# Schaudge/cellranger

Measured on AMD Instinct MI355X. Metric: M reads/sec barcode-correct+UMI-count, higher is better.
Workload: dtype u32/u64 integer keys; f64 posterior

## Files before the change

cellranger_amd/csrc/dedup.hip:

```cpp
#include "block_utils.h"
#include "common.h"

int cr_scan_small(crgpu_ctx *ctx, uint32_t *d_data, uint64_t n, uint32_t *d_total_out);
int cr_partition_by_owner(crgpu_ctx *ctx, const uint64_t *d_in, uint64_t *d_out, uint64_t n, uint32_t sh_bc,
                          uint32_t n_ranks, const uint32_t *bounds, uint64_t *counts_out);

#define NONE32 0xFFFFFFFFu

struct crgpu_counts {
    uint64_t n_triplets = 0, n_molecules = 0;
    uint32_t *d_bc = nullptr, *d_feature = nullptr, *d_count = nullptr;
    uint64_t *d_mkeys = nullptr;
    uint32_t *d_mreads = nullptr;
    uint32_t *d_corr_reads = nullptr;
    uint32_t *d_filt_reads = nullptr;
    int32_t *d_mprobe = nullptr;
    uint32_t *d_back = nullptr;
    uint32_t n_back = 0;
    uint32_t n_canon = 0;
    KeyLayout layout;
    bool pt_valid = false;
    uint32_t pt_n_probes = 0;
    uint64_t n_pt = 0;
    uint32_t *d_pt_bc = nullptr, *d_pt_probe = nullptr, *d_pt_count = nullptr;
// ... 709 lines not shown
}
__device__ __forceinline__ uint32_t rep_source(uint32_t min_raw, uint32_t K, uint32_t sK) {
    return (min_raw != 0xFFFFFFFFu && (min_raw < K || (sK & ST_CORRECTED))) ? min_raw : 0xFFFFFFFFu;
}

struct TargetFilter {
    const uint8_t *on_target;
    uint32_t n_features, sh_feat, bits_feat;
    uint64_t min_reads;
    __device__ __forceinline__ bool filtered(uint64_t key, uint32_t read_count, bool low) const {
        if (!min_reads) return false;
        const uint32_t f = (uint32_t)((key >> sh_feat) & lowmask(bits_feat));
        return f < n_features && on_target[f] != 0 && (uint64_t)read_count < min_reads && !low;
    }
};
struct MolFlag {
    const uint16_t *st;
    __device__ __forceinline__ bool operator()(uint64_t k) const {
        const uint32_t s = st[k];
        const bool landed = !(s & ST_CORRECTED) | (st_inc1(s) > 0u);
        return landed & !(s & ST_LOW);
    }
};
struct MolFlagTargeted {
    const uint16_t *st;
    const uint64_t *ukey;
    const uint32_t *upos, *inc_all;
    uint64_t n_keys, n_dist;
    TargetFilter tf;
    __device__ __forceinline__ bool operator()(uint64_t k) const {
        const uint32_t s = st[k];
        const bool landed = !(s & ST_CORRECTED) | (st_inc1(s) > 0u);
        if (!landed || (s & ST_LOW)) return false;
        const uint32_t end = k + 1 < n_dist ? upos[k + 1] : (uint32_t)n_keys;
        const uint32_t rc = ((s & ST_CORRECTED) ? 0u : end - upos[k]) + (st_inc1(s) ? inc_all[k] : 0u);
        return !tf.filtered(ukey[k], rc, false);
    }
};
struct EmitMol {
    const uint64_t *ukey;
    const uint32_t *upos, *inc_all, *minidx;
    const uint16_t *st;
    uint64_t n_keys, n_dist;
    uint64_t *mkeys;
    uint32_t *mreads;
    const uint32_t *rep_read = nullptr;
    const int32_t *probe = nullptr;
    int32_t *mprobe = nullptr;
    struct Pre {
        uint64_t key;
        uint32_t p0, p1, s;
    };
    __device__ __forceinline__ Pre pre(uint64_t k) const {
        Pre p;
        p.key = ukey[k];
        p.p0 = upos[k];
        p.p1 = upos[k + 1 < n_dist ? k + 1 : k];
        p.s = st[k];
        return p;
    }
    __device__ __forceinline__ Pre pre_own(uint64_t k) const {
        Pre p;
        p.key = ukey[k];
        p.p0 = upos[k];
        p.p1 = 0u;
        p.s = st[k];
        return p;
    }
    __device__ __forceinline__ void operator()(uint64_t k, uint32_t o, const Pre &p) const {
        uint32_t inc = 0u, mi = NONE32;
        if (st_inc1(p.s)) {
            inc = inc_all[k];
            mi = rep_source(minidx[k], (uint32_t)k, p.s);
        }
        const uint64_t bit = (mi != NONE32 ? ukey[mi] : p.key) & 1ull;
        mkeys[o] = (p.key & ~1ull) | bit;
        const uint32_t end = k + 1 < n_dist ? p.p1 : (uint32_t)n_keys;
        const uint32_t cnt = end - p.p0;
        mreads[o] = ((p.s & ST_CORRECTED) ? 0u : cnt) + inc;
        if (mprobe) mprobe[o] = probe[rep_read[mi != NONE32 ? mi : (uint32_t)k]];
    }
};

__device__ __forceinline__ bool rl_is_head(uint64_t key, uint64_t &carry_key, bool &carry_valid, uint32_t shift, uint32_t lane) {
    uint64_t left = __shfl_up(key, 1);
    if (lane == 0) left = carry_key;
    const bool head = (lane == 0 && !carry_valid) || (key >> shift) != (left >> shift);
    carry_key = __shfl(key, 63);
    carry_valid = true;
    return head;
}

__global__ __launch_bounds__(CP_BLOCK) void k_rl_count(const uint64_t *__restrict__ keys, const uint32_t shift, const uint64_t n,
                                                       const uint64_t tile, uint32_t *__restrict__ block_counts) {
    __shared__ uint32_t ws[CP_WAVES];
    const uint32_t lane = threadIdx.x & 63u, wave = threadIdx.x >> 6;
    const uint64_t lo = (uint64_t)blockIdx.x * tile;
    const uint64_t hi = lo + tile < n ? lo + tile : n;
    uint32_t c = 0;
    for (uint64_t base = lo; base < hi; base += CP_ROUND) {
        uint64_t key[CP_ITEMS];
        const uint64_t w0 = base + (uint64_t)wave * (64u * CP_ITEMS);
        const uint64_t wb = w0 > 0 ? (w0 - 1 < n ? w0 - 1 : n - 1) : 0;
        uint64_t carry_key = keys[wb];
        bool carry_valid = w0 > 0;
#pragma unroll
        for (int j = 0; j < CP_ITEMS; j++) {
            const uint64_t i = w0 + (uint64_t)j * 64 + lane;
            key[j] = keys[i < hi ? i : hi - 1];
        }
#pragma unroll
        for (int j = 0; j < CP_ITEMS; j++) {
            const uint64_t i = w0 + (uint64_t)j * 64 + lane;
            const bool head = rl_is_head(key[j], carry_key, carry_valid, shift, lane);
            c += (head && i < hi) ? 1u : 0u;
        }
    }
#pragma unroll
    for (int d = 32; d >= 1; d >>= 1) c += __shfl_xor(c, d);
    if (lane == 0) ws[wave] = c;
    __syncthreads();
    if (threadIdx.x == 0) {
        uint32_t t = 0;
        for (int w = 0; w < CP_WAVES; w++) t += ws[w];
        block_counts[blockIdx.x] = t;
    }
}

__global__ __launch_bounds__(CP_BLOCK) void k_rl_write(const uint64_t *__restrict__ keys, const uint32_t shift, const uint64_t n,
                                                       const uint64_t tile, const uint32_t *__restrict__ block_offs,
                                                       uint64_t *__restrict__ ukey, uint32_t *__restrict__ upos) {
    __shared__ uint32_t ws[CP_ITEMS * CP_WAVES];
    __shared__ uint32_t round_total;
    const uint32_t lane = threadIdx.x & 63u, wave = threadIdx.x >> 6;
    const uint64_t lo = (uint64_t)blockIdx.x * tile;
    const uint64_t hi = lo + tile < n ? lo + tile : n;
    uint32_t run = block_offs[blockIdx.x];
    for (uint64_t base = lo; base < hi; base += CP_ROUND) {
        uint64_t key[CP_ITEMS];
        bool f[CP_ITEMS];
        uint32_t below[CP_ITEMS];
        const uint64_t w0 = base + (uint64_t)wave * (64u * CP_ITEMS);
        const uint64_t wb = w0 > 0 ? (w0 - 1 < n ? w0 - 1 : n - 1) : 0;
        uint64_t carry_key = keys[wb];
        bool carry_valid = w0 > 0;
#pragma unroll
        for (int j = 0; j < CP_ITEMS; j++) {
            const uint64_t i = w0 + (uint64_t)j * 64 + lane;
            key[j] = keys[i < hi ? i : hi - 1];
        }
#pragma unroll
        for (int j = 0; j < CP_ITEMS; j++) {
            const uint64_t i = w0 + (uint64_t)j * 64 + lane;
            f[j] = rl_is_head(key[j], carry_key, carry_valid, shift, lane) && i < hi;
            const unsigned long long m = __ballot(f[j]);
            below[j] = (uint32_t)__popcll(m & ((1ull << lane) - 1ull));
            if (lane == 0) ws[wave * CP_ITEMS + j] = (uint32_t)__popcll(m);
        }
        __syncthreads();
        if (threadIdx.x < CP_ITEMS * CP_WAVES) {
            const uint32_t v = ws[threadIdx.x];
            uint32_t x = v;
#pragma unroll
            for (int d = 1; d < CP_ITEMS * CP_WAVES; d <<= 1) {
                const uint32_t y = __shfl_up(x, d);
                if (threadIdx.x >= (uint32_t)d) x += y;
            }
            ws[threadIdx.x] = x - v;
            if (threadIdx.x == CP_ITEMS * CP_WAVES - 1) round_total = x;
        }
        __syncthreads();
#pragma unroll
        for (int j = 0; j < CP_ITEMS; j++)
            if (f[j]) {
                const uint32_t o = run + ws[wave * CP_ITEMS + j] + below[j];
                ukey[o] = key[j];
                upos[o] = (uint32_t)(w0 + (uint64_t)j * 64 + lane);
            }
        run += round_total;
        __syncthreads();
    }
}

static int run_lengths(crgpu_ctx *ctx, const uint64_t *keys, uint32_t shift, uint64_t n, uint64_t *ukey, uint32_t *upos,
                       uint32_t *d_block, uint32_t *d_total_out, bool counts_ready = false) {
    uint64_t tile;
    const uint32_t nb = cp_blocks(n, &tile);
    if (!counts_ready)
        hipLaunchKernelGGL(k_rl_count, dim3(nb), dim3(CP_BLOCK), 0, ctx->stream, keys, shift, n, tile, d_block);
    else
        ctx->rl_counts_from_finish++;
    CR_TRY(cr_scan_small(ctx, d_block, nb, d_total_out));
    hipLaunchKernelGGL(k_rl_write, dim3(nb), dim3(CP_BLOCK), 0, ctx->stream, keys, shift, n, tile, d_block, ukey, upos);
    CR_HIP(ctx, hipGetLastError());
    return CRGPU_OK;
}

struct MtCarry {
    uint64_t prefix;
    bool has_mol;
    bool valid;
};

template <typename Flag>
__device__ __forceinline__ MtCarry mt_carry_from_memory(const Flag &flag, const uint64_t *__restrict__ ukey, uint32_t sh_feat,
                                                        uint64_t nd, uint64_t i0) {
    MtCarry c{0ull, false, false};
    if (i0 == 0 || i0 >= nd) return c;
    c.valid = true;
    uint64_t p = i0 - 1;
    c.prefix = ukey[p] >> sh_feat;
    c.has_mol = flag(p);
    while (!c.has_mol && p > 0) {
        p--;
        if ((ukey[p] >> sh_feat) != c.prefix) break;
        c.has_mol = flag(p);
    }
    return c;
}

__device__ __forceinline__ bool mt_opens_triplet(bool is_mol, uint64_t key, uint32_t sh_feat, uint32_t lane, MtCarry &carry) {
    const uint64_t prefix = key >> sh_feat;
    const uint64_t left = __shfl_up(prefix, 1);
    const unsigned long long starts = __ballot(lane == 0 || prefix != left), mols = __ballot(is_mol);
    const unsigned long long upto = ~0ull >> (63u - lane);
    const uint32_t rs = 63u - (uint32_t)__clzll((long long)(starts & upto));
    const unsigned long long between = (upto >> 1) & ~((1ull << rs) - 1ull);
    const uint64_t prefix0 = __shfl(prefix, 0);
    const bool carried = carry.valid && carry.prefix == prefix0 && carry.has_mol;
    const bool open = (mols & between) == 0ull && !(rs == 0u && carried);
    const uint32_t rs_last = 63u - (uint32_t)__clzll((long long)starts);
    const bool last_has = (mols >> rs_last) != 0ull || (rs_last == 0u && carried);
    carry.prefix = __shfl(prefix, 63);
    carry.has_mol = last_has;
    carry.valid = true;
    return is_mol && open;
}

#define MT_WAVE_SPAN (64u * CP_ITEMS)
template <typename Flag>
__global__ __launch_bounds__(CP_BLOCK) void k_mt_count(const Flag flag, const uint64_t *__restrict__ ukey, const uint32_t sh_feat,
                                                       const uint64_t nd, const uint64_t tile, uint32_t *__restrict__ mol_counts,
                                                       uint32_t *__restrict__ head_counts) {
    __shared__ uint32_t ws[2 * CP_WAVES];
    const uint32_t lane = threadIdx.x & 63u, wave = threadIdx.x >> 6;
    const uint64_t lo = (uint64_t)blockIdx.x * tile;
    const uint64_t hi = lo + tile < nd ? lo + tile : nd;
    uint32_t cm = 0, ch = 0;
    for (uint64_t base = lo; base < hi; base += CP_ROUND) {
        bool f[CP_ITEMS];
        uint64_t key[CP_ITEMS];
        const uint64_t w0 = base + (uint64_t)wave * MT_WAVE_SPAN;
#pragma unroll
        for (int j = 0; j < CP_ITEMS; j++) {
            const uint64_t i = w0 + (uint64_t)j * 64 + lane;
            const uint64_t ic = i < hi ? i : hi - 1;
            f[j] = flag(ic);
            key[j] = ukey[ic];
        }
        MtCarry carry = mt_carry_from_memory(flag, ukey, sh_feat, nd, w0);
#pragma unroll
        for (int j = 0; j < CP_ITEMS; j++) {
            const uint64_t i = w0 + (uint64_t)j * 64 + lane;
            const bool m = f[j] && i < hi;
            const bool h = mt_opens_triplet(m, key[j], sh_feat, lane, carry);
            cm += m ? 1u : 0u;
            ch += h ? 1u : 0u;
        }
    }
#pragma unroll
    for (int d = 32; d >= 1; d >>= 1) {
        cm += __shfl_xor(cm, d);
        ch += __shfl_xor(ch, d);
    }
    if (lane == 0) {
        ws[wave] = cm;
// ... 70 lines not shown
            ws[threadIdx.x] = x - v;
            if (threadIdx.x == CP_ITEMS * CP_WAVES - 1) round_total = x;
        }
        __syncthreads();
#pragma unroll
        for (int j = 0; j < CP_ITEMS; j++)
            if (f[j]) {
                const uint64_t i = w0 + (uint64_t)j * 64 + lane;
                const uint32_t w = ws[wave * CP_ITEMS + j];
                const uint32_t o = run_m + (w & 0xFFFFu) + below_m[j];
                emit(i, o, pre[j]);
                if (h[j]) {
                    const uint32_t t = run_h + (w >> 16) + below_h[j];
                    const uint32_t bcf = (uint32_t)(pre[j].key >> sh_bc);
                    tbc[t] = back ? back[bcf] : bcf;
                    tfeat[t] = (uint32_t)((pre[j].key >> sh_feat) & lowmask(bits_feat));
                    tpos[t] = o;
                }
            }
        run_m += round_total & 0xFFFFu;
        run_h += round_total >> 16;
        __syncthreads();
    }
}

__global__ __launch_bounds__(256) void k_trip_counts(const uint32_t *__restrict__ tpos, uint64_t nt, uint64_t nm,
                                                     uint32_t *__restrict__ cnt) {
    const uint64_t stride = (uint64_t)gridDim.x * blockDim.x;
    for (uint64_t t = (uint64_t)blockIdx.x * blockDim.x + threadIdx.x; t < nt; t += stride)
        cnt[t] = (t + 1 < nt ? tpos[t + 1] : (uint32_t)nm) - tpos[t];
}

__device__ __forceinline__ void segment_bounds(const uint64_t *__restrict__ ukey, uint64_t nd, uint64_t k, uint32_t shift,
                                               uint64_t &s, uint64_t &e) {
    const uint64_t pre = ukey[k] >> shift;
    uint64_t lo = k, step = 1;
    while (lo >= step && (ukey[lo - step] >> shift) == pre) {
        lo -= step;
        step <<= 1;
    }
    uint64_t a = lo >= step ? lo - step + 1 : 0, b = lo;
    while (a < b) {
        const uint64_t mid = (a + b) >> 1;
        if ((ukey[mid] >> shift) == pre) b = mid; else a = mid + 1;
    }
    s = a;
    uint64_t hi = k;
    step = 1;
    while (hi + step < nd && (ukey[hi + step] >> shift) == pre) {
        hi += step;
        step <<= 1;
    }
    a = hi;
    b = hi + step < nd ? hi + step - 1 : nd - 1;
    while (a < b) {
        const uint64_t mid = (a + b + 1) >> 1;
        if ((ukey[mid] >> shift) == pre) a = mid; else b = mid - 1;
    }
    e = a + 1;
}

__device__ __forceinline__ uint32_t run_count(const uint32_t *__restrict__ upos, uint64_t nd, uint64_t n_keys, uint64_t k) {
    const uint32_t end = k + 1 < nd ? upos[k + 1] : (uint32_t)n_keys;
    return end - upos[k];
}

#include "umi_correct.h"

__device__ __forceinline__ uint64_t group_id(const KL &kl, uint64_t key) {
    const uint64_t umi = (key >> kl.sh_umi) & lowmask(kl.bits_umi);
    const uint64_t lib = (key >> kl.sh_lib) & lowmask(kl.bits_lib + kl.bits_ulen);
    const uint64_t bc = key >> kl.sh_bc;
    return ((bc << (kl.bits_lib + kl.bits_ulen)) | lib) << kl.bits_umi | umi;
}
__device__ __forceinline__ uint32_t group_hash(uint64_t g) {
    g ^= g >> 33;
    g *= 0xff51afd7ed558ccdull;
    g ^= g >> 33;
    g *= 0xc4ceb9fe1a85ec53ull;
    g ^= g >> 33;
    return (uint32_t)g;
}

#define LF_TILE 8192u
#define LF_ENTRY_BITS 18u
#define LF_WORDS (1u << (LF_ENTRY_BITS - 4u))
__device__ __forceinline__ uint64_t mix64(uint64_t g) {
    g ^= g >> 33;
    g *= 0xff51afd7ed558ccdull;
    g ^= g >> 33;
    g *= 0xc4ceb9fe1a85ec53ull;
    g ^= g >> 33;
    return g;
}
#define LF_THREADS 1024u
#define LF_BATCH 4
#define LS_HASH_BITS 32u
__device__ __forceinline__ void lf_note(uint32_t *bm, uint32_t e) {
    const uint32_t sh = (e & 15u) * 2u;
    const uint32_t old = atomicOr(&bm[e >> 4], 1u << sh);
    if ((old >> sh) & 1u) atomicOr(&bm[e >> 4], 2u << sh);
}
__device__ __forceinline__ bool lf_again(const uint32_t *bm, uint32_t e) { return (bm[e >> 4] >> ((e & 15u) * 2u + 1u)) & 1u; }
__global__ __launch_bounds__(LF_THREADS) void k_group_candidates(const KL kl, const uint64_t *__restrict__ ukey, uint64_t nd,
                                                                 uint8_t *__restrict__ cand) {
    __shared__ uint32_t bm[LF_WORDS];
    __shared__ uint32_t s_first;
    __shared__ unsigned long long s_end;
    const uint32_t tid = threadIdx.x;
    const uint64_t n_tiles = (nd + LF_TILE - 1) / LF_TILE;
    const uint32_t emask = (1u << LF_ENTRY_BITS) - 1u;
    for (uint64_t tile = blockIdx.x; tile < n_tiles; tile += gridDim.x) {
        const uint64_t t0 = tile * LF_TILE;
        const uint64_t t1 = t0 + LF_TILE < nd ? t0 + LF_TILE : nd;
        if (tid == 0) s_first = 0xFFFFFFFFu;
        for (uint32_t w = tid; w < LF_WORDS; w += LF_THREADS) bm[w] = 0u;
        __syncthreads();
        {
            uint32_t mine = 0xFFFFFFFFu;
#pragma unroll
            for (uint32_t j = 0; j < LF_TILE / LF_THREADS; j++) {
                const uint64_t p = t0 + j * LF_THREADS + tid;
                if (p < t1 && mine == 0xFFFFFFFFu && (p == 0 || (ukey[p] >> kl.sh_bc) != (ukey[p - 1] >> kl.sh_bc)))
                    mine = (uint32_t)(p - t0);
            }
            if (mine != 0xFFFFFFFFu) atomicMin(&s_first, mine);
        }
        __syncthreads();
        const uint32_t first = s_first;
        if (tid == 0) {
            uint64_t b = nd;
            if (first != 0xFFFFFFFFu && t1 < nd) {
                const uint64_t bcv = ukey[t1 - 1] >> kl.sh_bc;
                uint64_t lo = t1 - 1, step = 1;
                while (lo + step < nd && (ukey[lo + step] >> kl.sh_bc) == bcv) {
                    lo += step;
                    step <<= 1;
                }
                uint64_t hi = lo + step < nd ? lo + step : nd;
                while (lo + 1 < hi) {
                    const uint64_t mid = (lo + hi) >> 1;
                    if ((ukey[mid] >> kl.sh_bc) == bcv) lo = mid; else hi = mid;
                }
                b = hi;
            }
            s_end = b;
        }
        __syncthreads();
        if (first == 0xFFFFFFFFu) continue;
        const uint64_t a = t0 + first, b = s_end;
        for (uint64_t k0 = a + tid; k0 < b; k0 += (uint64_t)LF_THREADS * LF_BATCH) {
            uint64_t key[LF_BATCH];
#pragma unroll
            for (int j = 0; j < LF_BATCH; j++) {
                const uint64_t k = k0 + (uint64_t)j * LF_THREADS;
                key[j] = k < b ? ukey[k] : 0ull;
            }
#pragma unroll
            for (int j = 0; j < LF_BATCH; j++) {
                if (k0 + (uint64_t)j * LF_THREADS >= b) break;
                lf_note(bm, (uint32_t)mix64(group_id(kl, key[j])) & emask);
            }
        }
        __syncthreads();
        for (uint64_t k0 = a + tid; k0 < b; k0 += (uint64_t)LF_THREADS * LF_BATCH) {
            uint64_t key[LF_BATCH];
#pragma unroll
            for (int j = 0; j < LF_BATCH; j++) {
                const uint64_t k = k0 + (uint64_t)j * LF_THREADS;
                key[j] = k < b ? ukey[k] : 0ull;
            }
#pragma unroll
            for (int j = 0; j < LF_BATCH; j++) {
                const uint64_t k = k0 + (uint64_t)j * LF_THREADS;
                if (k >= b) break;
                cand[k] = (uint8_t)lf_again(bm, (uint32_t)mix64(group_id(kl, key[j])) & emask);
            }
        }
        __syncthreads();
    }
}
struct CandFlag {
    const uint8_t *cand;
    __device__ __forceinline__ bool operator()(uint64_t k) const { return cand[k] != 0; }
};
struct EmitHash {
    KL kl;
    const uint64_t *ukey;
    uint32_t vbits;
    uint32_t *hash, *val;
    typedef uint64_t Pre;
    __device__ __forceinline__ Pre pre(uint64_t k) const { return ukey[k]; }
    __device__ __forceinline__ void operator()(uint64_t k, uint32_t o, Pre key) const {
        const uint64_t g = mix64(group_id(kl, key) ^ 0x9E3779B97F4A7C15ull);
        hash[o] = LS_HASH_BITS >= 32u ? (uint32_t)g : ((uint32_t)g & ((1u << (LS_HASH_BITS & 31u)) - 1u));
        const uint32_t extra = vbits >= 32u ? 0u : ((uint32_t)(g >> 32) << vbits);
        val[o] = extra | (uint32_t)k;
    }
};

__global__ __launch_bounds__(256) void k_low_support(const KL kl, const uint32_t *__restrict__ hash,
                                                     const uint32_t *__restrict__ val, uint64_t n_cand, uint64_t nd,
                                                     uint32_t vbits,
                                                     const uint64_t *__restrict__ ukey,
                                                     const uint32_t *__restrict__ upos, uint64_t n_keys,
                                                     uint16_t *__restrict__ st) {
    const uint64_t stride = (uint64_t)gridDim.x * blockDim.x;
    for (uint64_t j = (uint64_t)blockIdx.x * blockDim.x + threadIdx.x; j < n_cand; j += stride) {
        const uint32_t h = hash[j];
        const bool same_prev = j > 0 && hash[j - 1] == h;
        const bool same_next = j + 1 < n_cand && hash[j + 1] == h;
        if (!same_prev && !same_next) continue;
        uint64_t s = j, e = j + 1;
        while (s > 0 && hash[s - 1] == h) s--;
        while (e < n_cand && hash[e] == h) e++;
        const uint32_t vmask = vbits >= 32u ? 0xFFFFFFFFu : ((1u << vbits) - 1u);
        const uint32_t my_val = val[j];
        bool any = false;
        for (uint64_t t = s; t < e; t++) any |= t != j && ((val[t] ^ my_val) & ~vmask) == 0u;
        if (!any) continue;
        const uint32_t me = my_val & vmask;
        const uint64_t g = group_id(kl, ukey[me]);
        const uint32_t my_s = st[me];
        const uint32_t my_c1 = run_count(upos, nd, n_keys, me) - ((my_s & ST_CORRECTED) ? 1u : 0u) + st_inc1(my_s);
        uint32_t mx = my_c1, n_members = 0, n_max = 0;
        for (uint64_t t = s; t < e; t++) {
            if (((val[t] ^ my_val) & ~vmask) != 0u) continue;
            const uint32_t k = val[t] & vmask;
            if (group_id(kl, ukey[k]) != g) continue;
            const uint32_t ks = st[k];
            const uint32_t c1 = run_count(upos, nd, n_keys, k) - ((ks & ST_CORRECTED) ? 1u : 0u) + st_inc1(ks);
            n_members++;
            if (c1 > mx) {
                mx = c1;
                n_max = 1;
            } else if (c1 == mx) {
                n_max++;
            }
        }
        if (n_members < 2) continue;
        if (my_c1 < mx || n_max >= 2) st_or(st, me, ST_LOW);
    }
}

__global__ __launch_bounds__(256) void k_rep_read(const uint64_t *__restrict__ keys, const uint32_t *__restrict__ vals,
                                                  const uint32_t *__restrict__ upos, uint64_t nd, uint64_t n_keys,
                                                  uint32_t *__restrict__ rep_read) {
    const uint64_t stride = (uint64_t)gridDim.x * blockDim.x;
    for (uint64_t k = (uint64_t)blockIdx.x * blockDim.x + threadIdx.x; k < nd; k += stride) {
        const uint32_t b = upos[k], e = k + 1 < nd ? upos[k + 1] : (uint32_t)n_keys;
        const uint64_t bit = keys[b] & 1ull;
        uint32_t best = vals[b];
        for (uint32_t i = b + 1; i < e && (keys[i] & 1ull) == bit; i++) best = vals[i] < best ? vals[i] : best;
        rep_read[k] = best;
    }
}

struct __attribute__((aligned(4))) DupRec {
    uint32_t umi, read_count, flags;
};

struct __attribute__((aligned(8))) DupRec8 {
    uint32_t umi_flags, read_count;
};
template <bool PACK8>
__global__ __launch_bounds__(256) void k_per_read(const KL kl, const uint64_t *__restrict__ ukey, const uint32_t *__restrict__ vals,
                                                  const uint32_t *__restrict__ upos, uint64_t nd, uint64_t n_keys,
                                                  const uint32_t *__restrict__ corr, const uint32_t *__restrict__ inc_all,
                                                  const uint16_t *__restrict__ st, const uint32_t *__restrict__ minidx,
                                                  const uint32_t *__restrict__ rep_read, void *__restrict__ packed_v,
                                                  const TargetFilter tf) {
    DupRec *__restrict__ packed = reinterpret_cast<DupRec *>(packed_v);
    DupRec8 *__restrict__ packed8 = reinterpret_cast<DupRec8 *>(packed_v);
    const uint64_t stride = (uint64_t)gridDim.x * blockDim.x;
    for (uint64_t k = (uint64_t)blockIdx.x * blockDim.x + threadIdx.x; k < nd; k += stride) {
        const uint32_t b = upos[k], e = k + 1 < nd ? upos[k + 1] : (uint32_t)n_keys;
        const bool corrected = (st[k] & ST_CORRECTED) != 0u;
        const uint32_t K = corrected ? corr[k] : (uint32_t)k;
        const uint32_t sK = st[K];
        const uint32_t endK = (uint64_t)K + 1 < nd ? upos[K + 1] : (uint32_t)n_keys;
        const uint32_t cntK = endK - upos[K];
        const bool is_target = st_inc1(sK) != 0u;
// ... 205 lines not shown
            ctx->timing = was_timing;
        }
        if (t0) {
            ctx->event_pool.push_back(t0);
            ctx->event_pool.push_back(t1);
        }
    }
};

static int count_keys_impl(crgpu_ctx *ctx, uint64_t *d_keys_inout, uint64_t n_keys, crgpu_counts **out, PerRead pr) {
    if (!ctx || !out) return CRGPU_EINVAL;
    *out = nullptr;
    CR_REQUIRE(ctx, ctx->layout.set, CRGPU_ESTATE, "crgpu_count_keys: call crgpu_set_key_layout first");
    CR_REQUIRE(ctx, n_keys <= 0x7FFFFFFFull, CRGPU_ERANGE, "crgpu_count_keys: at most 2^31-1 keys per call");
    CR_TRY(cr_dense_ensure(ctx));
    const KeyLayout &L = ctx->layout;
    const KL kl = make_kl(L);
    crgpu_counts *res = new (std::nothrow) crgpu_counts();
    if (!res) return cr_fail(ctx, CRGPU_ENOMEM, "out of host memory");
    res->layout = L;
    res->n_canon = ctx->n_canon;
    if (n_keys == 0) {
        *out = res;
        return CRGPU_OK;
    }
    CR_REQUIRE(ctx, L.total_bits() <= 64, CRGPU_ESTATE,
               "crgpu_count_keys: the key layout needs the dense barcode index (CRGPU_OPT_DENSE_BARCODE_KEYS) and none is valid -- "
               "were the keys built before the last change of a histogram table?");
    CR_REQUIRE(ctx, d_keys_inout, CRGPU_EINVAL, "crgpu_count_keys: NULL keys");
    struct Guard {
        crgpu_ctx *c;
        crgpu_counts *r;
        bool armed = true;
        ~Guard() {
            if (armed) crgpu_counts_free(c, r);
        }
    } guard{ctx, res};

    uint32_t *d_block = ctx->d_sort_hist;
    uint32_t *d_total = ctx->d_scalars + 16;
    if (ctx->dense.valid) {
        res->n_back = ctx->dense.V;
        CR_TRY(cr_pool_alloc(ctx, (void **)&res->d_back, (size_t)ctx->dense.V * sizeof(uint32_t)));
        CR_HIP(ctx, hipMemcpyAsync(res->d_back, ctx->dense.d_back, (size_t)ctx->dense.V * sizeof(uint32_t), hipMemcpyDeviceToDevice,
                                   ctx->stream));
    }

    DevBuf tmp, vtmp;
    CR_TRY(dmalloc(ctx, tmp, n_keys * sizeof(uint64_t)));
    if (pr.d_vals) CR_TRY(dmalloc(ctx, vtmp, n_keys * sizeof(uint32_t)));
    bool in_tmp = false;
    uint32_t low_left = 0;
    CR_TRY(cr_radix_sort_u64_top(ctx, d_keys_inout, tmp.as<uint64_t>(), pr.d_vals, pr.d_vals ? vtmp.as<uint32_t>() : nullptr, n_keys,
                                 L.total_bits(), &in_tmp, &low_left));
    uint64_t *keys_rw = in_tmp ? tmp.as<uint64_t>() : d_keys_inout;
    uint32_t *vals_rw = pr.d_vals ? (in_tmp ? vtmp.as<uint32_t>() : pr.d_vals) : nullptr;

    DevBuf ukey_b, upos_b;
    CR_TRY(dmalloc(ctx, ukey_b, n_keys * sizeof(uint64_t)));
    CR_TRY(dmalloc(ctx, upos_b, (n_keys + 1) * sizeof(uint32_t)));
    uint64_t *ukey = ukey_b.as<uint64_t>();
    uint32_t *upos = upos_b.as<uint32_t>();
    CrRunHeads rl_heads{1u, 0, d_block, false};
    if (low_left) {
        bool fell_back = false;
        (void)cp_blocks(n_keys, &rl_heads.tile);
        CR_TRY(cr_order_runs(ctx, keys_rw, vals_rw, n_keys, low_left, &fell_back, &rl_heads));
        if (fell_back) {
            ctx->sort_refinished++;
            uint64_t *other = in_tmp ? d_keys_inout : tmp.as<uint64_t>();
            uint32_t *vother = pr.d_vals ? (in_tmp ? pr.d_vals : vtmp.as<uint32_t>()) : nullptr;
            bool flip = false;
            CR_TRY(cr_radix_sort_u64_full(ctx, keys_rw, other, vals_rw, vother, n_keys, L.total_bits(), &flip));
            if (flip) {
                keys_rw = other;
                vals_rw = vother;
            }
            rl_heads.valid = false;
        }
    }
    const uint64_t *keys = keys_rw;
    const uint32_t *vals = vals_rw;
    uint32_t nd32 = 0;
    {
        CrTimer t(ctx, CRGPU_T_DEDUP, n_keys);
        CR_TRY(run_lengths(ctx, keys, 1u, n_keys, ukey, upos, d_block, d_total, rl_heads.valid));
    }
    CR_TRY(read_u32(ctx, d_total, &nd32));
    const uint64_t nd = nd32;

    const uint64_t st_bytes = ((nd + 1) & ~1ull) * sizeof(uint16_t) + 4;
    DevBuf corr_b, incall_b, st_b, minidx_b;
    CR_TRY(dmalloc(ctx, minidx_b, nd * sizeof(uint32_t)));
    CR_TRY(dmalloc(ctx, corr_b, nd * sizeof(uint32_t)));
    CR_TRY(dmalloc(ctx, incall_b, nd * sizeof(uint32_t)));
    CR_TRY(dmalloc(ctx, st_b, st_bytes));
    uint32_t *corr = corr_b.as<uint32_t>(), *inc_all = incall_b.as<uint32_t>(), *minidx = minidx_b.as<uint32_t>();
    uint16_t *st = st_b.as<uint16_t>();
    const bool overlap = CrFork::enabled(ctx, nd);
    CrFork fork(ctx);
    DevBuf heads_b, giant_b, best_b;
    if (overlap) CR_TRY(fork.mark());
    {
        const bool timing_was = ctx->timing;
        if (overlap) ctx->timing = false;
        struct TimingBack {
            crgpu_ctx *c;
            bool v;
            ~TimingBack() { c->timing = v; }
        } timing_back{ctx, timing_was};
        CrTimer t(ctx, CRGPU_T_DEDUP);
        CR_HIP(ctx, hipMemsetAsync(inc_all, 0, nd * sizeof(uint32_t), ctx->stream));
        CR_HIP(ctx, hipMemsetAsync(st, 0, st_bytes, ctx->stream));
        CR_HIP(ctx, hipMemsetAsync(minidx, 0xFF, nd * sizeof(uint32_t), ctx->stream));
        const uint64_t n_tiles = (nd + UC_TILE - 1) / UC_TILE;
        CR_TRY(dmalloc(ctx, heads_b, 2 * n_tiles * sizeof(uint32_t)));
        uint32_t *tile_first = heads_b.as<uint32_t>(), *tile_last = tile_first + n_tiles;
#ifndef UC_GRID_WG
#define UC_GRID_WG 5u
#endif
        hipLaunchKernelGGL(k_correct_umis_tiled, dim3(cr_grid(n_tiles, 1, 256u * UC_GRID_WG)), dim3(256), 0, ctx->stream, kl, ukey,
                           upos, nd, n_keys, tile_first, tile_last, corr, st, inc_all, minidx);
        if (n_tiles > 1) {
            const size_t lds_small = (2 * UES_CAP + UES_BUCKETS * 8) * sizeof(uint32_t);
            const size_t lds_large = (2 * UE_CAP + UE_BUCKETS * 8) * sizeof(uint32_t);
            cr_allow_lds(ctx, (const void *)k_correct_umis_edges<false>, lds_large);
            cr_allow_lds(ctx, (const void *)k_giant_probe, lds_large);
            const uint64_t max_items = nd / (UE_CAP / 2) + 16;
            CR_TRY(dmalloc(ctx, giant_b, max_items * sizeof(GiantItem) + 16));
            CR_TRY(dmalloc(ctx, best_b, nd * sizeof(unsigned long long)));
            uint32_t *n_giant = reinterpret_cast<uint32_t *>(giant_b.as<unsigned char>());
            GiantItem *items = reinterpret_cast<GiantItem *>(giant_b.as<unsigned char>() + 16);
            unsigned long long *best = best_b.as<unsigned long long>();
            CR_HIP(ctx, hipMemsetAsync(n_giant, 0, sizeof(uint32_t), ctx->stream));
            hipLaunchKernelGGL(k_correct_umis_edges<true>, dim3(cr_grid(n_tiles - 1, 1, 256u * 6u)), dim3(UES_THREADS), lds_small,
                               ctx->stream, kl, ukey, upos, nd, n_keys, tile_first, tile_last, corr, st, inc_all, minidx, items, n_giant);
            hipLaunchKernelGGL(k_correct_umis_edges<false>, dim3(cr_grid(n_tiles - 1, 1, 256u * 2u)), dim3(UE_THREADS),
                               lds_large, ctx->stream, kl, ukey, upos, nd, n_keys, tile_first, tile_last, corr, st, inc_all,
                               minidx, items, n_giant);
            hipLaunchKernelGGL(k_giant_init, dim3(512), dim3(UE_THREADS), 0, ctx->stream, kl, ukey, upos, nd, n_keys, items,
                               n_giant, best);
            hipLaunchKernelGGL(k_giant_probe, dim3(512), dim3(UE_THREADS), lds_large, ctx->stream, kl, ukey, upos, nd, n_keys,
                               items, n_giant, best);
            hipLaunchKernelGGL(k_giant_final, dim3(512), dim3(UE_THREADS), 0, ctx->stream, upos, nd, n_keys, items, n_giant, best,
                               corr, st, inc_all, minidx);
        }
        CR_HIP(ctx, hipGetLastError());
    }

    {
        DevBuf cand_b, h_b, v_b;
        CR_TRY(dmalloc(ctx, cand_b, nd));
        CR_TRY(dmalloc(ctx, h_b, nd * sizeof(uint32_t)));
        CR_TRY(dmalloc(ctx, v_b, nd * sizeof(uint32_t)));
        const uint32_t vbits = cr_ceil_log2(nd ? nd : 1);
        uint32_t n_cand32 = 0;
        if (overlap) CR_TRY(fork.side(fork.t0));
        {
            CrTimer t(ctx, CRGPU_T_DEDUP);
            const uint64_t n_ftiles = (nd + LF_TILE - 1) / LF_TILE;
            hipLaunchKernelGGL(k_group_candidates, dim3(cr_grid(n_ftiles, 1, 256u * 2u)), dim3(LF_THREADS), 0, ctx->stream, kl, ukey, nd,
                               cand_b.as<uint8_t>());
            CR_HIP(ctx, hipGetLastError());
            CR_TRY(compact(ctx, CandFlag{cand_b.as<uint8_t>()}, EmitHash{kl, ukey, vbits, h_b.as<uint32_t>(), v_b.as<uint32_t>()}, nd, d_block,
                           d_total));
        }
        CR_TRY(read_u32(ctx, d_total, &n_cand32));
        const uint64_t n_cand = n_cand32;
        ctx->last_distinct_keys = nd;
        ctx->last_low_support_candidates = n_cand;
        if (n_cand >= 2) {
            DevBuf ht_b, vt_b;
            CR_TRY(dmalloc(ctx, ht_b, n_cand * sizeof(uint32_t)));
            CR_TRY(dmalloc(ctx, vt_b, n_cand * sizeof(uint32_t)));
            bool s_in_tmp = false;
            CR_TRY(cr_radix_sort_u32(ctx, h_b.as<uint32_t>(), ht_b.as<uint32_t>(), v_b.as<uint32_t>(), vt_b.as<uint32_t>(), n_cand,
                                     0, LS_HASH_BITS, &s_in_tmp));
            CR_TRY(fork.join());
            {
                CrTimer t(ctx, CRGPU_T_DEDUP);
                hipLaunchKernelGGL(k_low_support, dim3(cr_grid(n_cand, 256)), dim3(256), 0, ctx->stream, kl,
                                   s_in_tmp ? ht_b.as<uint32_t>() : h_b.as<uint32_t>(),
                                   s_in_tmp ? vt_b.as<uint32_t>() : v_b.as<uint32_t>(), n_cand, nd, vbits, ukey, upos, n_keys, st);
                CR_HIP(ctx, hipGetLastError());
            }
        }
        CR_TRY(fork.join());
    }

    const TargetFilter tf{ctx->d_on_target, ctx->n_target_features, L.sh_feat(), L.bits_feat, ctx->d_on_target ? ctx->target_min_reads : 0};
    CrFork fork2(ctx);
    DevBuf rep_b, packed_b;
    const bool want_probe = vals && pr.d_probe;
    if (vals) CR_TRY(dmalloc(ctx, rep_b, nd * sizeof(uint32_t)));
    if (want_probe) {
        CrTimer t(ctx, CRGPU_T_DEDUP);
        hipLaunchKernelGGL(k_rep_read, dim3(cr_grid(nd, 256)), dim3(256), 0, ctx->stream, keys, vals, upos, nd, n_keys,
                           rep_b.as<uint32_t>());
        CR_HIP(ctx, hipGetLastError());
    }
    if (vals && CrFork::enabled(ctx, nd)) {
        CR_TRY(fork2.mark());
        CR_TRY(fork2.side(fork2.t0));
    }
    const uint32_t side_wgs = fork2.on_side ? 256u * 6u : 256u * 8u;
    if (vals) {
        CrTimer t(ctx, CRGPU_T_DEDUP);
        if (!want_probe)
            hipLaunchKernelGGL(k_rep_read, dim3(cr_grid(nd, 256, side_wgs)), dim3(256), 0, ctx->stream, keys, vals, upos, nd, n_keys,
                               rep_b.as<uint32_t>());
        if (pr.packed_out) CR_HIP(ctx, hipMemsetAsync(pr.packed_out, 0, pr.n_reads * sizeof(DupRec), ctx->stream));
        const bool pack8 = !pr.packed_out && kl.bits_umi <= 24u;
        if (!pr.packed_out) {
            const uint64_t bytes = pr.n_reads * (pack8 ? sizeof(DupRec8) : sizeof(DupRec));
            CR_TRY(dmalloc(ctx, packed_b, bytes));
            CR_HIP(ctx, hipMemsetAsync(packed_b.p, 0, bytes, ctx->stream));
        }
        DupRec *packed = pr.packed_out ? pr.packed_out : packed_b.as<DupRec>();
        if (pack8)
            hipLaunchKernelGGL(k_per_read<true>, dim3(cr_grid(nd, 256, side_wgs)), dim3(256), 0, ctx->stream, kl, ukey, vals, upos, nd, n_keys,
                               corr, inc_all, st, minidx, rep_b.as<uint32_t>(), (void *)packed, tf);
        else
            hipLaunchKernelGGL(k_per_read<false>, dim3(cr_grid(nd, 256, side_wgs)), dim3(256), 0, ctx->stream, kl, ukey, vals, upos, nd, n_keys,
                               corr, inc_all, st, minidx, rep_b.as<uint32_t>(), (void *)packed, tf);
        if (!pr.packed_out) {
            if (pack8)
                hipLaunchKernelGGL(k_unpack_dupinfo<true>, dim3(cr_grid(pr.n_reads, 256, side_wgs)), dim3(256), 0, ctx->stream,
                                   (const void *)packed, pr.n_reads, pr.out_umi, pr.out_cnt, pr.out_flags);
            else
                hipLaunchKernelGGL(k_unpack_dupinfo<false>, dim3(cr_grid(pr.n_reads, 256, side_wgs)), dim3(256), 0, ctx->stream,
                                   (const void *)packed, pr.n_reads, pr.out_umi, pr.out_cnt, pr.out_flags);
        }
        CR_HIP(ctx, hipGetLastError());
    }
    fork2.pause();

    DevBuf mkeys_b, mreads_b, tpos_b;
    CR_TRY(dmalloc(ctx, mkeys_b, nd * sizeof(uint64_t)));
    CR_TRY(dmalloc(ctx, mreads_b, nd * sizeof(uint32_t)));
    uint32_t nm32 = 0, nt32 = 0;
    if (want_probe) CR_TRY(cr_pool_alloc(ctx, (void **)&res->d_mprobe, nd * sizeof(int32_t)));
    CR_TRY(dmalloc(ctx, tpos_b, (nd + 1) * sizeof(uint32_t)));
    CR_TRY(cr_pool_alloc(ctx, (void **)&res->d_bc, nd * sizeof(uint32_t)));
    CR_TRY(cr_pool_alloc(ctx, (void **)&res->d_feature, nd * sizeof(uint32_t)));
    uint32_t *d_heads = d_block + 4096;
    uint32_t *d_total_h = ctx->d_scalars + 17;
    {
        CrTimer t(ctx, CRGPU_T_DEDUP);
// ... 875 lines not shown
```

Measured before the change: 17500.

## Record barcode-group starts during run-length write and use atomic candidate append

The run-length write kernel now also marks barcode boundaries and records, for each LF tile of the distinct-key array, the first barcode-group start via atomicMin. The group-candidate kernel reads these precomputed starts instead of rescanning ukey and doing a galloping search for each tile's end. The ordered two-pass compaction of candidates is replaced by a single-pass kernel that loads packed flag bytes and appends through a global atomic counter. Candidate order therefore becomes nondeterministic, which is acceptable only because the candidates are radix-sorted by hash afterwards; it adds a memset and extra atomics in the write kernel.

Result: slower. 17130 (-2.1%).

```diff
diff --git a/cellranger_amd/csrc/dedup.hip b/cellranger_amd/csrc/dedup.hip
--- a/cellranger_amd/csrc/dedup.hip
+++ b/cellranger_amd/csrc/dedup.hip
@@ -815,14 +815,19 @@
     }
 };
 
-__device__ __forceinline__ bool rl_is_head(uint64_t key, uint64_t &carry_key, bool &carry_valid, uint32_t shift, uint32_t lane) {
+__device__ __forceinline__ bool rl_is_head(uint64_t key, uint64_t &carry_key, bool &carry_valid, uint32_t shift, uint32_t lane,
+                                           uint32_t sh_bc = 0, bool *bc_head = nullptr) {
     uint64_t left = __shfl_up(key, 1);
     if (lane == 0) left = carry_key;
-    const bool head = (lane == 0 && !carry_valid) || (key >> shift) != (left >> shift);
+    const bool no_left = lane == 0 && !carry_valid;
+    const bool head = no_left || (key >> shift) != (left >> shift);
+    if (bc_head) *bc_head = no_left || (key >> sh_bc) != (left >> sh_bc);
     carry_key = __shfl(key, 63);
     carry_valid = true;
     return head;
 }
+
+#define LF_TILE 8192u
 
 __global__ __launch_bounds__(CP_BLOCK) void k_rl_count(const uint64_t *__restrict__ keys, const uint32_t shift, const uint64_t n,
                                                        const uint64_t tile, uint32_t *__restrict__ block_counts) {
@@ -862,7 +867,8 @@
 
 __global__ __launch_bounds__(CP_BLOCK) void k_rl_write(const uint64_t *__restrict__ keys, const uint32_t shift, const uint64_t n,
                                                        const uint64_t tile, const uint32_t *__restrict__ block_offs,
-                                                       uint64_t *__restrict__ ukey, uint32_t *__restrict__ upos) {
+                                                       uint64_t *__restrict__ ukey, uint32_t *__restrict__ upos,
+                                                       const uint32_t sh_bc, uint32_t *__restrict__ bc_first) {
     __shared__ uint32_t ws[CP_ITEMS * CP_WAVES];
     __shared__ uint32_t round_total;
     const uint32_t lane = threadIdx.x & 63u, wave = threadIdx.x >> 6;
@@ -871,7 +877,7 @@
     uint32_t run = block_offs[blockIdx.x];
     for (uint64_t base = lo; base < hi; base += CP_ROUND) {
         uint64_t key[CP_ITEMS];
-        bool f[CP_ITEMS];
+        bool f[CP_ITEMS], bh[CP_ITEMS];
         uint32_t below[CP_ITEMS];
         const uint64_t w0 = base + (uint64_t)wave * (64u * CP_ITEMS);
         const uint64_t wb = w0 > 0 ? (w0 - 1 < n ? w0 - 1 : n - 1) : 0;
@@ -885,7 +891,7 @@
 #pragma unroll
         for (int j = 0; j < CP_ITEMS; j++) {
             const uint64_t i = w0 + (uint64_t)j * 64 + lane;
-            f[j] = rl_is_head(key[j], carry_key, carry_valid, shift, lane) && i < hi;
+            f[j] = rl_is_head(key[j], carry_key, carry_valid, shift, lane, sh_bc, &bh[j]) && i < hi;
             const unsigned long long m = __ballot(f[j]);
             below[j] = (uint32_t)__popcll(m & ((1ull << lane) - 1ull));
             if (lane == 0) ws[wave * CP_ITEMS + j] = (uint32_t)__popcll(m);
@@ -909,6 +915,7 @@
                 const uint32_t o = run + ws[wave * CP_ITEMS + j] + below[j];
                 ukey[o] = key[j];
                 upos[o] = (uint32_t)(w0 + (uint64_t)j * 64 + lane);
+                if (bc_first && bh[j]) atomicMin(&bc_first[o / LF_TILE], o);
             }
         run += round_total;
         __syncthreads();
@@ -916,15 +923,18 @@
 }
 
 static int run_lengths(crgpu_ctx *ctx, const uint64_t *keys, uint32_t shift, uint64_t n, uint64_t *ukey, uint32_t *upos,
-                       uint32_t *d_block, uint32_t *d_total_out, bool counts_ready = false) {
+                       uint32_t *d_block, uint32_t *d_total_out, bool counts_ready = false, uint32_t sh_bc = 0,
+                       uint32_t *bc_first = nullptr) {
     uint64_t tile;
     const uint32_t nb = cp_blocks(n, &tile);
+    if (bc_first) CR_HIP(ctx, hipMemsetAsync(bc_first, 0xFF, (n + LF_TILE - 1) / LF_TILE * sizeof(uint32_t), ctx->stream));
     if (!counts_ready)
         hipLaunchKernelGGL(k_rl_count, dim3(nb), dim3(CP_BLOCK), 0, ctx->stream, keys, shift, n, tile, d_block);
     else
         ctx->rl_counts_from_finish++;
     CR_TRY(cr_scan_small(ctx, d_block, nb, d_total_out));
-    hipLaunchKernelGGL(k_rl_write, dim3(nb), dim3(CP_BLOCK), 0, ctx->stream, keys, shift, n, tile, d_block, ukey, upos);
+    hipLaunchKernelGGL(k_rl_write, dim3(nb), dim3(CP_BLOCK), 0, ctx->stream, keys, shift, n, tile, d_block, ukey, upos, sh_bc,
+                       bc_first);
     CR_HIP(ctx, hipGetLastError());
     return CRGPU_OK;
 }
@@ -1161,7 +1171,6 @@
     return (uint32_t)g;
 }
 
-#define LF_TILE 8192u
 #define LF_ENTRY_BITS 18u
 #define LF_WORDS (1u << (LF_ENTRY_BITS - 4u))
 __device__ __forceinline__ uint64_t mix64(uint64_t g) {
@@ -1182,52 +1191,30 @@
 }
 __device__ __forceinline__ bool lf_again(const uint32_t *bm, uint32_t e) { return (bm[e >> 4] >> ((e & 15u) * 2u + 1u)) & 1u; }
 __global__ __launch_bounds__(LF_THREADS) void k_group_candidates(const KL kl, const uint64_t *__restrict__ ukey, uint64_t nd,
-                                                                 uint8_t *__restrict__ cand) {
+                                                                 const uint32_t *__restrict__ bc_first, uint8_t *__restrict__ cand) {
     __shared__ uint32_t bm[LF_WORDS];
-    __shared__ uint32_t s_first;
-    __shared__ unsigned long long s_end;
+    __shared__ uint32_t s_end;
     const uint32_t tid = threadIdx.x;
     const uint64_t n_tiles = (nd + LF_TILE - 1) / LF_TILE;
     const uint32_t emask = (1u << LF_ENTRY_BITS) - 1u;
     for (uint64_t tile = blockIdx.x; tile < n_tiles; tile += gridDim.x) {
-        const uint64_t t0 = tile * LF_TILE;
-        const uint64_t t1 = t0 + LF_TILE < nd ? t0 + LF_TILE : nd;
-        if (tid == 0) s_first = 0xFFFFFFFFu;
+        const uint32_t first = bc_first[tile];
+        if (first == 0xFFFFFFFFu) continue;
         for (uint32_t w = tid; w < LF_WORDS; w += LF_THREADS) bm[w] = 0u;
+        if (tid < 64u) {
+            uint32_t e = (uint32_t)nd;
+            for (uint64_t t = tile + 1; t < n_tiles; t += 64) {
+                const uint32_t v = t + tid < n_tiles ? bc_first[t + tid] : 0xFFFFFFFFu;
+                const unsigned long long m = __ballot(v != 0xFFFFFFFFu);
+                if (m) {
+                    e = __shfl(v, __ffsll(m) - 1);
+                    break;
+                }
+            }
+            if (tid == 0) s_end = e;
+        }
         __syncthreads();
-        {
-            uint32_t mine = 0xFFFFFFFFu;
-#pragma unroll
-            for (uint32_t j = 0; j < LF_TILE / LF_THREADS; j++) {
-                const uint64_t p = t0 + j * LF_THREADS + tid;
-                if (p < t1 && mine == 0xFFFFFFFFu && (p == 0 || (ukey[p] >> kl.sh_bc) != (ukey[p - 1] >> kl.sh_bc)))
-                    mine = (uint32_t)(p - t0);
-            }
-            if (mine != 0xFFFFFFFFu) atomicMin(&s_first, mine);
-        }
-        __syncthreads();
-        const uint32_t first = s_first;
-        if (tid == 0) {
-            uint64_t b = nd;
-            if (first != 0xFFFFFFFFu && t1 < nd) {
-                const uint64_t bcv = ukey[t1 - 1] >> kl.sh_bc;
-                uint64_t lo = t1 - 1, step = 1;
-                while (lo + step < nd && (ukey[lo + step] >> kl.sh_bc) == bcv) {
-                    lo += step;
-                    step <<= 1;
-                }
-                uint64_t hi = lo + step < nd ? lo + step : nd;
-                while (lo + 1 < hi) {
-                    const uint64_t mid = (lo + hi) >> 1;
-                    if ((ukey[mid] >> kl.sh_bc) == bcv) lo = mid; else hi = mid;
-                }
-                b = hi;
-            }
-            s_end = b;
-        }
-        __syncthreads();
-        if (first == 0xFFFFFFFFu) continue;
-        const uint64_t a = t0 + first, b = s_end;
+        const uint64_t a = first, b = s_end;
         for (uint64_t k0 = a + tid; k0 < b; k0 += (uint64_t)LF_THREADS * LF_BATCH) {
             uint64_t key[LF_BATCH];
 #pragma unroll
@@ -1268,15 +1255,77 @@
     const uint64_t *ukey;
     uint32_t vbits;
     uint32_t *hash, *val;
-    typedef uint64_t Pre;
-    __device__ __forceinline__ Pre pre(uint64_t k) const { return ukey[k]; }
-    __device__ __forceinline__ void operator()(uint64_t k, uint32_t o, Pre key) const {
+    __device__ __forceinline__ void operator()(uint64_t k, uint32_t o, uint64_t key) const {
         const uint64_t g = mix64(group_id(kl, key) ^ 0x9E3779B97F4A7C15ull);
         hash[o] = LS_HASH_BITS >= 32u ? (uint32_t)g : ((uint32_t)g & ((1u << (LS_HASH_BITS & 31u)) - 1u));
         const uint32_t extra = vbits >= 32u ? 0u : ((uint32_t)(g >> 32) << vbits);
         val[o] = extra | (uint32_t)k;
     }
 };
+
+#define CA_ROUNDS 16
+#define CA_WAVE_SPAN (64u * 8u * CA_ROUNDS)
+#define CA_TILE (4u * CA_WAVE_SPAN)
+__global__ __launch_bounds__(256) void k_cand_append(const EmitHash emit, const uint8_t *__restrict__ cand, const uint64_t nd,
+                                                     uint32_t *__restrict__ counter) {
+    __shared__ uint32_t ws[4];
+    __shared__ uint32_t s_base;
+    const uint32_t lane = threadIdx.x & 63u, wave = threadIdx.x >> 6;
+    const uint64_t w0 = (uint64_t)blockIdx.x * CA_TILE + (uint64_t)wave * CA_WAVE_SPAN + lane * 8u;
+    uint64_t f8[CA_ROUNDS];
+#pragma unroll
+    for (int r = 0; r < CA_ROUNDS; r++) {
+        const uint64_t k = w0 + (uint64_t)r * 512u;
+        f8[r] = 0;
+        if (k + 8 <= nd) {
+            f8[r] = *reinterpret_cast<const uint64_t *>(cand + k);
+        } else {
+            for (uint32_t j = 0; j < 8u; j++)
+                if (k + j < nd) f8[r] |= (uint64_t)cand[k + j] << (8u * j);
+        }
+    }
+    uint32_t mask[CA_ROUNDS / 4] = {};
+    uint32_t c = 0;
+#pragma unroll
+    for (int r = 0; r < CA_ROUNDS; r++) {
+        const uint32_t m8 = (uint32_t)((f8[r] * 0x0102040810204080ull) >> 56);
+        mask[r >> 2] |= m8 << ((r & 3) * 8);
+        c += (uint32_t)__popc(m8);
+    }
+#pragma unroll
+    for (int d = 32; d >= 1; d >>= 1) c += __shfl_xor(c, d);
+    if (lane == 0) ws[wave] = c;
+    __syncthreads();
+    if (threadIdx.x == 0) {
+        const uint32_t t = ws[0] + ws[1] + ws[2] + ws[3];
+        s_base = t ? atomicAdd(counter, t) : 0u;
+    }
+    __syncthreads();
+    uint32_t run = s_base;
+    for (uint32_t w = 0; w < wave; w++) run += ws[w];
+    if (c == 0) return;
+#pragma unroll 2
+    for (int r = 0; r < CA_ROUNDS; r++) {
+        const uint32_t m8 = (mask[r >> 2] >> ((r & 3) * 8)) & 0xFFu;
+        if (__ballot(m8 != 0u) == 0ull) continue;
+        const uint64_t k = w0 + (uint64_t)r * 512u;
+        uint64_t key[8];
+#pragma unroll
+        for (int j = 0; j < 8; j++) key[j] = ((m8 >> j) & 1u) ? emit.ukey[k + j] : 0ull;
+        const uint32_t n_mine = (uint32_t)__popc(m8);
+        uint32_t x = n_mine;
+#pragma unroll
+        for (int d = 1; d < 64; d <<= 1) {
+            const uint32_t y = __shfl_up(x, d);
+            if (lane >= (uint32_t)d) x += y;
+        }
+        uint32_t o = run + x - n_mine;
+        run += __shfl(x, 63);
+#pragma unroll
+        for (int j = 0; j < 8; j++)
+            if ((m8 >> j) & 1u) emit(k + j, o++, key[j]);
+    }
+}
 
 __global__ __launch_bounds__(256) void k_low_support(const KL kl, const uint32_t *__restrict__ hash,
                                                      const uint32_t *__restrict__ val, uint64_t n_cand, uint64_t nd,
@@ -1648,9 +1697,11 @@
     const uint64_t *keys = keys_rw;
     const uint32_t *vals = vals_rw;
     uint32_t nd32 = 0;
+    DevBuf bc_first_b;
+    CR_TRY(dmalloc(ctx, bc_first_b, (n_keys + LF_TILE - 1) / LF_TILE * sizeof(uint32_t)));
     {
         CrTimer t(ctx, CRGPU_T_DEDUP, n_keys);
-        CR_TRY(run_lengths(ctx, keys, 1u, n_keys, ukey, upos, d_block, d_total, rl_heads.valid));
+        CR_TRY(run_lengths(ctx, keys, 1u, n_keys, ukey, upos, d_block, d_total, rl_heads.valid, kl.sh_bc, bc_first_b.as<uint32_t>()));
     }
     CR_TRY(read_u32(ctx, d_total, &nd32));
     const uint64_t nd = nd32;
@@ -1725,11 +1776,12 @@
         {
             CrTimer t(ctx, CRGPU_T_DEDUP);
             const uint64_t n_ftiles = (nd + LF_TILE - 1) / LF_TILE;
+            CR_HIP(ctx, hipMemsetAsync(d_total, 0, sizeof(uint32_t), ctx->stream));
             hipLaunchKernelGGL(k_group_candidates, dim3(cr_grid(n_ftiles, 1, 256u * 2u)), dim3(LF_THREADS), 0, ctx->stream, kl, ukey, nd,
-                               cand_b.as<uint8_t>());
+                               bc_first_b.as<uint32_t>(), cand_b.as<uint8_t>());
+            hipLaunchKernelGGL(k_cand_append, dim3((uint32_t)((nd + CA_TILE - 1) / CA_TILE)), dim3(256), 0, ctx->stream,
+                               EmitHash{kl, ukey, vbits, h_b.as<uint32_t>(), v_b.as<uint32_t>()}, cand_b.as<uint8_t>(), nd, d_total);
             CR_HIP(ctx, hipGetLastError());
-            CR_TRY(compact(ctx, CandFlag{cand_b.as<uint8_t>()}, EmitHash{kl, ukey, vbits, h_b.as<uint32_t>(), v_b.as<uint32_t>()}, nd, d_block,
-                           d_total));
         }
         CR_TRY(read_u32(ctx, d_total, &n_cand32));
         const uint64_t n_cand = n_cand32;
```
